# sonbui25/Multimodal-Aspect-Category-Sentiment-Analysis

Hardware: AMD Instinct MI355X
Metric: train samples/sec (fwd+bwd+step) FCMF seq128x36ROI (higher is better)
Workload: dtype bf16; 1 GPU; FCMF-base fine-tune step, BASELINE configs[1]: batch 64 reviews x 6 aspects per GPU, seq 128, 7 images x (49 patches + 36 ROIs), precomputed ResNet-152 features, dropout 0.1, clip 1.0 + 4-group AdamW + linear schedule; global_batch=64, per_gpu_batch=64, seq_len=128, parallelism=dp1, sample_unit=1 review = 6 aspect forwards

## Files before the change

### multimodal-aspect-category-sentiment-analysis_amd/csrc/norm.hip

```cpp
#include "common.h"

constexpr int LN_MAXP = 8;

template <typename T, int NP>
__global__ __launch_bounds__(256) void add_ln_fwd_kernel(const T* __restrict__ x, const T* __restrict__ res,
                                                         int64_t res_stride, const float* __restrict__ gamma,
                                                         const float* __restrict__ beta, T* __restrict__ y,
                                                         T* __restrict__ z, float* __restrict__ mean,
                                                         float* __restrict__ rstd, int rows, int H, float eps,
                                                         float p, uint64_t seed, unsigned char* __restrict__ q8 = nullptr,
                                                         float* __restrict__ qscale = nullptr) {
  const int lane = threadIdx.x & 63;
  const float inv_keep = p > 0.f ? 1.0f / (1.0f - p) : 1.0f;
  typedef typename Vec4<T>::raw Raw;
  const int stride = gridDim.x * 4;
  int row = blockIdx.x * 4 + (threadIdx.x >> 6);
  Raw nx[NP], nr[NP];
  auto fetch = [&](int r) {
    if (r < rows) {
#pragma unroll
      for (int i = 0; i < NP; ++i) {
        const int c = (i * 64 + lane) * 4;
        if (c < H) {
          nx[i] = Vec4<T>::load_raw(x + (int64_t)r * H + c);
          if (res) nr[i] = Vec4<T>::load_raw(res + (int64_t)r * res_stride + c);
        }
      }
    }
  };
  fetch(row);
  for (; row < rows; row += stride) {
  Raw cx[NP], cr[NP];
#pragma unroll
  for (int i = 0; i < NP; ++i) { cx[i] = nx[i]; cr[i] = nr[i]; }
  fetch(row + stride);
  float4 v[NP];
  float s = 0.f;
#pragma unroll
  for (int i = 0; i < NP; ++i) {
    const int c = (i * 64 + lane) * 4;
    if (c < H) {
      float4 a = Vec4<T>::cvt(cx[i]);
      if (p > 0.f) {
        const uint64_t base = (uint64_t)row * H + c;
        float dm[4];
        dropout_mult4(seed, base, p, inv_keep, dm);
        a.x *= dm[0]; a.y *= dm[1]; a.z *= dm[2]; a.w *= dm[3];
      }
      if (res) {
        float4 r = Vec4<T>::cvt(cr[i]);
        a.x += r.x; a.y += r.y; a.z += r.z; a.w += r.w;
      }
      v[i] = a;
      s += a.x + a.y + a.z + a.w;
    }
  }
  const float mu = wave_sum(s) / (float)H;
  float q = 0.f;
#pragma unroll
  for (int i = 0; i < NP; ++i) {
    const int c = (i * 64 + lane) * 4;
    if (c < H) {
      float dx = v[i].x - mu, dy = v[i].y - mu, dz = v[i].z - mu, dw = v[i].w - mu;
      q += dx * dx + dy * dy + dz * dz + dw * dw;
    }
  }
  const float rs = rsqrtf(wave_sum(q) / (float)H + eps);
  if (lane == 0) { mean[row] = mu; rstd[row] = rs; }
  float amax = 0.f;
#pragma unroll
  for (int i = 0; i < NP; ++i) {
    const int c = (i * 64 + lane) * 4;
    if (c < H) {
      if (z) Vec4<T>::store(z + (int64_t)row * H + c, v[i]);
      const float4 g = *reinterpret_cast<const float4*>(gamma + c);
      const float4 b = *reinterpret_cast<const float4*>(beta + c);
      float4 o;
      o.x = (v[i].x - mu) * rs * g.x + b.x; o.y = (v[i].y - mu) * rs * g.y + b.y;
      o.z = (v[i].z - mu) * rs * g.z + b.z; o.w = (v[i].w - mu) * rs * g.w + b.w;
      Vec4<T>::store(y + (int64_t)row * H + c, o);
      if (q8) {
        o.x = to_f32<T>(from_f32<T>(o.x)); o.y = to_f32<T>(from_f32<T>(o.y)); o.z = to_f32<T>(from_f32<T>(o.z)); o.w = to_f32<T>(from_f32<T>(o.w));
        v[i] = o;
        amax = fmaxf(amax, fmaxf(fmaxf(fabsf(o.x), fabsf(o.y)), fmaxf(fabsf(o.z), fabsf(o.w))));
      }
    }
  }
  if (q8) {
    amax = wave_max(amax);
    const float sc = amax > 0.f ? amax * (1.0f / 448.0f) : 1.0f, inv = 1.0f / sc;
    if (lane == 0) qscale[row] = sc;
#pragma unroll
    for (int i = 0; i < NP; ++i) {
      const int c = (i * 64 + lane) * 4;
      if (c < H) {
        int w8 = 0;
        w8 = __builtin_amdgcn_cvt_pk_fp8_f32(v[i].x * inv, v[i].y * inv, w8, false);
        w8 = __builtin_amdgcn_cvt_pk_fp8_f32(v[i].z * inv, v[i].w * inv, w8, true);
        *reinterpret_cast<int*>(q8 + (int64_t)row * H + c) = w8;
      }
    }
  }
  }
}

template <typename T, int NP>
__global__ __launch_bounds__(256) void add_ln_bwd_kernel(const T* __restrict__ dy, const T* __restrict__ z,
                                                         const float* __restrict__ gamma,
                                                         const float* __restrict__ mean,
                                                         const float* __restrict__ rstd, T* __restrict__ dz,
                                                         T* __restrict__ dx, float* __restrict__ dgamma,
                                                         float* __restrict__ dbeta, float* __restrict__ dxsum,
                                                         float* __restrict__ partial, int rows, int H, float p,
                                                         uint64_t seed, unsigned char* __restrict__ q8 = nullptr,
                                                         float* __restrict__ qscale = nullptr) {
  __shared__ float4 red[2][3][NP][64];
  const int lane = threadIdx.x & 63, w = threadIdx.x >> 6;
  const float inv_keep = p > 0.f ? 1.0f / (1.0f - p) : 1.0f;
  float4 ag[NP], ab[NP], gm[NP], ax[NP];
#pragma unroll
  for (int i = 0; i < NP; ++i) {
    ag[i] = make_float4(0, 0, 0, 0); ab[i] = make_float4(0, 0, 0, 0); ax[i] = make_float4(0, 0, 0, 0);
    const int c = (i * 64 + lane) * 4;
    gm[i] = c < H ? *reinterpret_cast<const float4*>(gamma + c) : make_float4(0, 0, 0, 0);
  }
  typedef typename Vec4<T>::raw Raw;
  const int stride = gridDim.x * 4;
  int row = blockIdx.x * 4 + w;
  Raw nd[NP], nz[NP];
  float nmu = 0.f, nrs = 0.f;
  auto fetch = [&](int r) {
    if (r < rows) {
      nmu = mean[r]; nrs = rstd[r];
#pragma unroll
      for (int i = 0; i < NP; ++i) {
        const int c = (i * 64 + lane) * 4;
        if (c < H) { nd[i] = Vec4<T>::load_raw(dy + (int64_t)r * H + c); nz[i] = Vec4<T>::load_raw(z + (int64_t)r * H + c); }
      }
    }
  };
  fetch(row);
  for (; row < rows; row += stride) {
    const float mu = nmu, rs = nrs;
    Raw cd[NP], cz[NP];
#pragma unroll
    for (int i = 0; i < NP; ++i) { cd[i] = nd[i]; cz[i] = nz[i]; }
    fetch(row + stride);
    float4 gy[NP], xh[NP];
    float s1 = 0.f, s2 = 0.f;
#pragma unroll
    for (int i = 0; i < NP; ++i) {
      const int c = (i * 64 + lane) * 4;
      if (c < H) {
        const float4 d = Vec4<T>::cvt(cd[i]);
        const float4 zz = Vec4<T>::cvt(cz[i]);
        float4 h; h.x = (zz.x - mu) * rs; h.y = (zz.y - mu) * rs; h.z = (zz.z - mu) * rs; h.w = (zz.w - mu) * rs;
        ag[i].x += d.x * h.x; ag[i].y += d.y * h.y; ag[i].z += d.z * h.z; ag[i].w += d.w * h.w;
        ab[i].x += d.x; ab[i].y += d.y; ab[i].z += d.z; ab[i].w += d.w;
        float4 g; g.x = d.x * gm[i].x; g.y = d.y * gm[i].y; g.z = d.z * gm[i].z; g.w = d.w * gm[i].w;
        gy[i] = g; xh[i] = h;
        s1 += g.x + g.y + g.z + g.w;
        s2 += g.x * h.x + g.y * h.y + g.z * h.z + g.w * h.w;
      }
    }
    s1 = wave_sum(s1) / (float)H;
    s2 = wave_sum(s2) / (float)H;
#pragma unroll
    for (int i = 0; i < NP; ++i) {
      const int c = (i * 64 + lane) * 4;
      if (c < H) {
        float4 o;
        o.x = rs * (gy[i].x - s1 - xh[i].x * s2); o.y = rs * (gy[i].y - s1 - xh[i].y * s2);
        o.z = rs * (gy[i].z - s1 - xh[i].z * s2); o.w = rs * (gy[i].w - s1 - xh[i].w * s2);
        Vec4<T>::store(dz + (int64_t)row * H + c, o);
        if (dx) {
          const uint64_t base = (uint64_t)row * H + c;
          float dm[4];
          dropout_mult4(seed, base, p, inv_keep, dm);
          o.x *= dm[0]; o.y *= dm[1]; o.z *= dm[2]; o.w *= dm[3];
          Vec4<T>::store(dx + (int64_t)row * H + c, o);
        }
        ax[i].x += o.x; ax[i].y += o.y; ax[i].z += o.z; ax[i].w += o.w;
        if (q8) {
          o.x = to_f32<T>(from_f32<T>(o.x)); o.y = to_f32<T>(from_f32<T>(o.y)); o.z = to_f32<T>(from_f32<T>(o.z)); o.w = to_f32<T>(from_f32<T>(o.w));
          gy[i] = o;
        }
      }
    }
    if (q8) {
      float amax = 0.f;
#pragma unroll
      for (int i = 0; i < NP; ++i)
        if ((i * 64 + lane) * 4 < H) amax = fmaxf(amax, fmaxf(fmaxf(fabsf(gy[i].x), fabsf(gy[i].y)), fmaxf(fabsf(gy[i].z), fabsf(gy[i].w))));
      amax = wave_max(amax);
      const float sc = amax > 0.f ? amax * (1.0f / 448.0f) : 1.0f, inv = 1.0f / sc;
      if (lane == 0) qscale[row] = sc;
#pragma unroll
      for (int i = 0; i < NP; ++i) {
        const int c = (i * 64 + lane) * 4;
        if (c < H) {
          int w8 = 0;
          w8 = __builtin_amdgcn_cvt_pk_fp8_f32(gy[i].x * inv, gy[i].y * inv, w8, false);
          w8 = __builtin_amdgcn_cvt_pk_fp8_f32(gy[i].z * inv, gy[i].w * inv, w8, true);
          *reinterpret_cast<int*>(q8 + (int64_t)row * H + c) = w8;
        }
      }
    }
  }
#pragma unroll
  for (int step = 0; step < 2; ++step) {
    const int half = step == 0 ? 2 : 1;
    if (w >= half && w < 2 * half) {
#pragma unroll
      for (int i = 0; i < NP; ++i) { red[w - half][0][i][lane] = ag[i]; red[w - half][1][i][lane] = ab[i]; red[w - half][2][i][lane] = ax[i]; }
    }
    __syncthreads();
    if (w < half) {
#pragma unroll
      for (int i = 0; i < NP; ++i) {
        float4 a = red[w][0][i][lane], b = red[w][1][i][lane], c2 = red[w][2][i][lane];
        ag[i].x += a.x; ag[i].y += a.y; ag[i].z += a.z; ag[i].w += a.w;
        ab[i].x += b.x; ab[i].y += b.y; ab[i].z += b.z; ab[i].w += b.w;
        ax[i].x += c2.x; ax[i].y += c2.y; ax[i].z += c2.z; ax[i].w += c2.w;
      }
    }
    __syncthreads();
  }
  if (w == 0) {
#pragma unroll
    for (int i = 0; i < NP; ++i) {
      const int c = (i * 64 + lane) * 4;
      if (c < H) {
        if (partial) {
          float* pb = partial + (int64_t)blockIdx.x * 3 * H + c;
          *reinterpret_cast<float4*>(pb) = ag[i];
          *reinterpret_cast<float4*>(pb + H) = ab[i];
          *reinterpret_cast<float4*>(pb + 2 * H) = ax[i];
        } else {
          atomicAdd(dgamma + c + 0, ag[i].x); atomicAdd(dgamma + c + 1, ag[i].y);
          atomicAdd(dgamma + c + 2, ag[i].z); atomicAdd(dgamma + c + 3, ag[i].w);
          atomicAdd(dbeta + c + 0, ab[i].x); atomicAdd(dbeta + c + 1, ab[i].y);
          atomicAdd(dbeta + c + 2, ab[i].z); atomicAdd(dbeta + c + 3, ab[i].w);
          if (dxsum) {
            atomicAdd(dxsum + c + 0, ax[i].x); atomicAdd(dxsum + c + 1, ax[i].y);
            atomicAdd(dxsum + c + 2, ax[i].z); atomicAdd(dxsum + c + 3, ax[i].w);
          }
        }
      }
    }
  }
}

__global__ __launch_bounds__(256) void ln_partial_reduce_kernel(const float* __restrict__ partial, int nblocks, int H,
                                                                float* __restrict__ dgamma, float* __restrict__ dbeta,
                                                                float* __restrict__ dxsum) {
  __shared__ float red[4][64];
  const int lane = threadIdx.x & 63, w = threadIdx.x >> 6;
  const int col = blockIdx.x * 64 + lane, which = blockIdx.y;
  float* out = which == 0 ? dgamma : (which == 1 ? dbeta : dxsum);
  if (!out) return;
  const int per = (nblocks + gridDim.z - 1) / gridDim.z;
  const int b0 = blockIdx.z * per, b1 = min(nblocks, b0 + per);
  float s = 0.f;
  if (col < H)
    for (int b = b0 + w; b < b1; b += 4) s += partial[((int64_t)b * 3 + which) * H + col];
  red[w][lane] = s;
  __syncthreads();
  if (w == 0 && col < H) atomicAdd(out + col, red[0][lane] + red[1][lane] + red[2][lane] + red[3][lane]);
}

__global__ __launch_bounds__(64) void position_ids_kernel(const int64_t* __restrict__ ids, int64_t* __restrict__ pos,
                                                          int S, int pad_id) {
  const int lane = threadIdx.x;
  const int64_t* row = ids + (int64_t)blockIdx.x * S;
  int64_t* out = pos + (int64_t)blockIdx.x * S;
  int running = 0;
  for (int t0 = 0; t0 < S; t0 += 64) {
    const int t = t0 + lane;
    const bool nz = t < S && row[t] != pad_id;
    const unsigned long long b = __ballot(nz);
    const int incl = __popcll(b & ((lane == 63) ? ~0ull : ((1ull << (lane + 1)) - 1)));
    if (t < S) out[t] = nz ? (int64_t)(running + incl + pad_id) : (int64_t)pad_id;
    running += __popcll(b);
  }
}

template <typename T, int NP>
__global__ __launch_bounds__(256) void embed_ln_fwd_kernel(const int64_t* __restrict__ ids, const int64_t* __restrict__ pos,
                                                           const int64_t* __restrict__ tt, const float* __restrict__ word,
                                                           const float* __restrict__ ptab, const float* __restrict__ ttab,
                                                           const float* __restrict__ gamma, const float* __restrict__ beta,
                                                           T* __restrict__ y, T* __restrict__ z, float* __restrict__ mean,
                                                           float* __restrict__ rstd, int ntok, int H, float eps, float p,
                                                           uint64_t seed) {
  const int lane = threadIdx.x & 63;
  const int row = blockIdx.x * 4 + (threadIdx.x >> 6);
  if (row >= ntok) return;
  const float* wr = word + ids[row] * H;
  const float* pr = ptab + pos[row] * H;
  const float* tr = ttab + (tt ? tt[row] : 0) * H;
  float4 v[NP];
  float s = 0.f;
#pragma unroll
  for (int i = 0; i < NP; ++i) {
    const int c = (i * 64 + lane) * 4;
    if (c < H) {
      const float4 a = *reinterpret_cast<const float4*>(wr + c);
      const float4 b = *reinterpret_cast<const float4*>(tr + c);
      const float4 d = *reinterpret_cast<const float4*>(pr + c);
      float4 o; o.x = (a.x + b.x) + d.x; o.y = (a.y + b.y) + d.y; o.z = (a.z + b.z) + d.z; o.w = (a.w + b.w) + d.w;
      v[i] = o;
      s += o.x + o.y + o.z + o.w;
    }
  }
  const float mu = wave_sum(s) / (float)H;
  float q = 0.f;
#pragma unroll
  for (int i = 0; i < NP; ++i) {
    const int c = (i * 64 + lane) * 4;
    if (c < H) {
      float dx = v[i].x - mu, dy = v[i].y - mu, dz = v[i].z - mu, dw = v[i].w - mu;
      q += dx * dx + dy * dy + dz * dz + dw * dw;
    }
  }
  const float rs = rsqrtf(wave_sum(q) / (float)H + eps);
  if (lane == 0) { mean[row] = mu; rstd[row] = rs; }
  const float inv_keep = p > 0.f ? 1.0f / (1.0f - p) : 1.0f;
#pragma unroll
  for (int i = 0; i < NP; ++i) {
    const int c = (i * 64 + lane) * 4;
    if (c < H) {
      if (z) Vec4<T>::store(z + (int64_t)row * H + c, v[i]);
      const float4 g = *reinterpret_cast<const float4*>(gamma + c);
      const float4 b = *reinterpret_cast<const float4*>(beta + c);
      float4 o;
      o.x = (v[i].x - mu) * rs * g.x + b.x; o.y = (v[i].y - mu) * rs * g.y + b.y;
      o.z = (v[i].z - mu) * rs * g.z + b.z; o.w = (v[i].w - mu) * rs * g.w + b.w;
      if (p > 0.f) {
        const uint64_t base = (uint64_t)row * H + c;
        float dm[4];
        dropout_mult4(seed, base, p, inv_keep, dm);
        o.x *= dm[0]; o.y *= dm[1]; o.z *= dm[2]; o.w *= dm[3];
      }
      Vec4<T>::store(y + (int64_t)row * H + c, o);
    }
  }
}

template <typename T>
__global__ __launch_bounds__(256) void embed_bwd_kernel(const T* __restrict__ dz, const int64_t* __restrict__ ids,
                                                        const int64_t* __restrict__ pos, const int64_t* __restrict__ tt,
                                                        float* __restrict__ dword, float* __restrict__ dpos,
                                                        float* __restrict__ dtt, int ntok, int H, int pad_id) {
  const int lane = threadIdx.x & 63;
  const int row = blockIdx.x * 4 + (threadIdx.x >> 6);
  if (row >= ntok) return;
  const int64_t id = ids[row], ps = pos[row], ty = tt ? tt[row] : 0;
  for (int c = lane; c < H; c += 64) {
    const float d = to_f32<T>(dz[(int64_t)row * H + c]);
    if (id != pad_id) atomicAdd(dword + id * H + c, d);
    if (dpos && ps != pad_id) atomicAdd(dpos + ps * H + c, d);
    if (dtt && ty != 0) atomicAdd(dtt + ty * H + c, d);
  }
}

template <typename T>
__global__ __launch_bounds__(256) void embed_type0_kernel(const T* __restrict__ dz, const int64_t* __restrict__ tt,
                                                          float* __restrict__ dtt, int ntok, int H, int rows_per_block) {
  __shared__ float red[4][64];
  const int lane = threadIdx.x & 63, w = threadIdx.x >> 6;
  const int col = blockIdx.x * 64 + lane;
  const int r0 = blockIdx.y * rows_per_block, r1 = min(ntok, r0 + rows_per_block);
  float s = 0.f;
  if (col < H)
    for (int r = r0 + w; r < r1; r += 4)
      if (!tt || tt[r] == 0) s += to_f32<T>(dz[(int64_t)r * H + col]);
  red[w][lane] = s;
  __syncthreads();
  if (w == 0 && col < H) atomicAdd(dtt + col, red[0][lane] + red[1][lane] + red[2][lane] + red[3][lane]);
}

template <typename T>
__global__ __launch_bounds__(256) void embed_pos_bwd_kernel(const T* __restrict__ dz, const int64_t* __restrict__ pos,
                                                            float* __restrict__ dpos, int nseq, int S, int H, int pad_id) {
  const int s = blockIdx.x, c = blockIdx.y * 256 + threadIdx.x;
  if (c >= H) return;
  int64_t p0 = -1;
  float acc = 0.f;
  const int g0 = blockIdx.z * 64, g1 = min(nseq, g0 + 64);
#pragma unroll 8
  for (int g = g0; g < g1; ++g) {
    const int64_t row = (int64_t)g * S + s, id = pos[row];
    if (id == pad_id) continue;
    const float d = to_f32<T>(dz[row * H + c]);
    if (p0 < 0) p0 = id;
    if (id == p0) acc += d;
    else atomicAdd(dpos + id * H + c, d);
  }
  if (p0 >= 0) atomicAdd(dpos + p0 * H + c, acc);
}

template <typename T>
__global__ __launch_bounds__(256) void embed_pos_type_bwd_kernel(const T* __restrict__ dz, const int64_t* __restrict__ pos,
                                                                 const int64_t* __restrict__ tt, float* __restrict__ dpos,
                                                                 float* __restrict__ dtt, int nseq, int S, int H, int pad_id) {
  constexpr int E = 16 / (int)sizeof(T);
  typedef T VecT __attribute__((ext_vector_type(E)));
  extern __shared__ __attribute__((aligned(16))) float red[];
  const int CE = H / E, slots = 256 / CE;
  const int tid = threadIdx.x, cg = tid % CE, slot = tid / CE, c0 = cg * E;
  const int s = blockIdx.x, g0 = blockIdx.y * 64, g1 = min(nseq, g0 + 64);
  float* rp = red;
  float* rt = red + slots * H;
  int* p0s = reinterpret_cast<int*>(red + 2 * slots * H);
  if (slot < slots) {
    float acc[E], tsum[E];
#pragma unroll
    for (int j = 0; j < E; ++j) acc[j] = tsum[j] = 0.f;
    int64_t p0 = -1;
#pragma unroll 4
    for (int g = g0 + slot; g < g1; g += slots) {
      const int64_t row = (int64_t)g * S + s, id = pos[row], ty = tt ? tt[row] : 0;
      const VecT v = *reinterpret_cast<const VecT*>(dz + row * H + c0);
      if (dtt) {
        if (ty == 0) {
#pragma unroll
          for (int j = 0; j < E; ++j) tsum[j] += (float)v[j];
        } else {
#pragma unroll
          for (int j = 0; j < E; ++j) atomicAdd(dtt + ty * H + c0 + j, (float)v[j]);
        }
      }
      if (id == pad_id) continue;
      if (p0 < 0) p0 = id;
      if (id == p0) {
#pragma unroll
        for (int j = 0; j < E; ++j) acc[j] += (float)v[j];
      } else {
#pragma unroll
        for (int j = 0; j < E; ++j) atomicAdd(dpos + id * H + c0 + j, (float)v[j]);
      }
    }
#pragma unroll
    for (int j = 0; j < E; ++j) { rp[slot * H + c0 + j] = acc[j]; rt[slot * H + c0 + j] = tsum[j]; }
    if (cg == 0) p0s[slot] = (int)p0;
  }
  __syncthreads();
  for (int c = tid; c < H; c += 256) {
    float ts = 0.f;
    for (int k = 0; k < slots; ++k) ts += rt[k * H + c];
    if (dtt) atomicAdd(dtt + c, ts);
    for (int k = 0; k < slots; ++k) {
      const int pk = p0s[k];
      if (pk < 0) continue;
      bool first = true;
      for (int m = 0; m < k; ++m) first = first && p0s[m] != pk;
      if (!first) continue;
      float ps = 0.f;
      for (int m = k; m < slots; ++m)
        if (p0s[m] == pk) ps += rp[m * H + c];
      atomicAdd(dpos + (int64_t)pk * H + c, ps);
    }
  }
}

#define LN_DISPATCH_T(T, H)                         \
  do {                                              \
    const int np__ = ((H) + 255) / 256;             \
    if (np__ <= 1) LAUNCH_(T, 1);                   \
    else if (np__ <= 2) LAUNCH_(T, 2);              \
    else if (np__ <= 3) LAUNCH_(T, 3);              \
    else if (np__ <= 4) LAUNCH_(T, 4);              \
    else LAUNCH_(T, 8);                             \
  } while (0)
#define LN_DISPATCH(dtype, H)                                     \
  do {                                                            \
    if ((dtype) == FCMF_F32) LN_DISPATCH_T(float, H);             \
    else LN_DISPATCH_T(bf16_t, H);                                \
  } while (0)

static int add_ln_fwd_impl(const void* x, const void* res, int64_t res_stride, const float* gamma, const float* beta, void* y,
                           void* z, float* mean, float* rstd, int rows, int H, float eps, float dropout_p, uint64_t seed,
                           int dtype, void* stream, void* q8, float* qscale);
extern "C" int fcmf_add_ln_fwd(const void* x, const void* res, int64_t res_stride, const float* gamma,
                               const float* beta, void* y, void* z, float* mean, float* rstd, int rows, int H,
                               float eps, float dropout_p, uint64_t seed, int dtype, void* stream) {
  return add_ln_fwd_impl(x, res, res_stride, gamma, beta, y, z, mean, rstd, rows, H, eps, dropout_p, seed, dtype, stream, nullptr, nullptr);
}
extern "C" int fcmf_add_ln_fwd_fp8(const void* x, const void* res, int64_t res_stride, const float* gamma,
                                   const float* beta, void* y, void* z, float* mean, float* rstd, int rows, int H,
                                   float eps, float dropout_p, uint64_t seed, int dtype, void* q8, float* qscale, void* stream) {
  if (!q8 || !qscale) return FCMF_ERR_ARG;
  return add_ln_fwd_impl(x, res, res_stride, gamma, beta, y, z, mean, rstd, rows, H, eps, dropout_p, seed, dtype, stream, q8, qscale);
}
static int add_ln_fwd_impl(const void* x, const void* res, int64_t res_stride, const float* gamma, const float* beta, void* y,
                           void* z, float* mean, float* rstd, int rows, int H, float eps, float dropout_p, uint64_t seed,
                           int dtype, void* stream, void* q8, float* qscale) {
  if (!x || !gamma || !beta || !y || !mean || !rstd || rows < 0 || H <= 0) return FCMF_ERR_ARG;
  if (H % 4 != 0 || H > LN_MAXP * 256 || (res && res_stride % 4 != 0)) return FCMF_ERR_UNSUPPORTED;
  if (rows == 0) return FCMF_OK;
  hipStream_t st = reinterpret_cast<hipStream_t>(stream);
  const int nblk = (rows + 3) / 4;
  dim3 grid(nblk > 2048 ? 2048 : nblk);
  if (dtype != FCMF_F32 && dtype != FCMF_BF16) return FCMF_ERR_UNSUPPORTED;
#define LAUNCH_(T, NP) hipLaunchKernelGGL((add_ln_fwd_kernel<T, NP>), grid, dim3(256), 0, st, (const T*)x, (const T*)res, \
    res_stride, gamma, beta, (T*)y, (T*)z, mean, rstd, rows, H, eps, dropout_p, seed, (unsigned char*)q8, qscale)
  LN_DISPATCH(dtype, H);
#undef LAUNCH_
  FCMF_CHECK_LAUNCH();
  return FCMF_OK;
}

static int ln_bwd_blocks(int rows) {
  int blocks = (rows + 3) / 4;
  return blocks > 1024 ? 1024 : blocks;
}

extern "C" int64_t fcmf_add_ln_bwd_workspace(int rows, int H) { return (int64_t)ln_bwd_blocks(rows) * 3 * H; }

static int add_ln_bwd_impl(const void* dy, const void* z, const float* gamma, const float* mean, const float* rstd, void* dz,
                           void* dx, float* dgamma, float* dbeta, float* dxsum, float* workspace, int rows, int H,
                           float dropout_p, uint64_t seed, int dtype, void* stream, void* q8, float* qscale);
extern "C" int fcmf_add_ln_bwd(const void* dy, const void* z, const float* gamma, const float* mean, const float* rstd,
                               void* dz, void* dx, float* dgamma, float* dbeta, float* dxsum, float* workspace,
                               int rows, int H, float dropout_p, uint64_t seed, int dtype, void* stream) {
  return add_ln_bwd_impl(dy, z, gamma, mean, rstd, dz, dx, dgamma, dbeta, dxsum, workspace, rows, H, dropout_p, seed, dtype, stream, nullptr, nullptr);
}
extern "C" int fcmf_add_ln_bwd_fp8(const void* dy, const void* z, const float* gamma, const float* mean, const float* rstd,
                                   void* dz, void* dx, float* dgamma, float* dbeta, float* dxsum, float* workspace,
                                   int rows, int H, float dropout_p, uint64_t seed, int dtype, void* q8, float* qscale, void* stream) {
  if (!q8 || !qscale) return FCMF_ERR_ARG;
  return add_ln_bwd_impl(dy, z, gamma, mean, rstd, dz, dx, dgamma, dbeta, dxsum, workspace, rows, H, dropout_p, seed, dtype, stream, q8, qscale);
}
static int add_ln_bwd_impl(const void* dy, const void* z, const float* gamma, const float* mean, const float* rstd, void* dz,
                           void* dx, float* dgamma, float* dbeta, float* dxsum, float* workspace, int rows, int H,
                           float dropout_p, uint64_t seed, int dtype, void* stream, void* q8, float* qscale) {
  if (!dy || !z || !gamma || !mean || !rstd || !dz || !dgamma || !dbeta || rows < 0 || H <= 0) return FCMF_ERR_ARG;
  if (H % 4 != 0 || H > LN_MAXP * 256) return FCMF_ERR_UNSUPPORTED;
  if (dropout_p > 0.f && !dx) return FCMF_ERR_ARG;
  if (rows == 0) return FCMF_OK;
  hipStream_t st = reinterpret_cast<hipStream_t>(stream);
  const int blocks = ln_bwd_blocks(rows);
  if (dtype != FCMF_F32 && dtype != FCMF_BF16) return FCMF_ERR_UNSUPPORTED;
#define LAUNCH_(T, NP) hipLaunchKernelGGL((add_ln_bwd_kernel<T, NP>), dim3(blocks), dim3(256), 0, st, (const T*)dy, (const T*)z, \
    gamma, mean, rstd, (T*)dz, (T*)(dropout_p > 0.f ? dx : nullptr), dgamma, dbeta, dxsum, workspace, rows, H, dropout_p, seed, \
    (unsigned char*)q8, qscale)
  LN_DISPATCH(dtype, H);
#undef LAUNCH_
  if (workspace)
    hipLaunchKernelGGL(ln_partial_reduce_kernel, dim3((H + 63) / 64, 3, 8), dim3(256), 0, st, workspace, blocks, H, dgamma, dbeta, dxsum);
  FCMF_CHECK_LAUNCH();
  return FCMF_OK;
}

extern "C" int fcmf_position_ids(const int64_t* ids, int64_t* pos, int nseq, int S, int pad_id, void* stream) {
  if (!ids || !pos || nseq < 0 || S <= 0) return FCMF_ERR_ARG;
  if (nseq == 0) return FCMF_OK;
  hipLaunchKernelGGL(position_ids_kernel, dim3(nseq), dim3(64), 0, reinterpret_cast<hipStream_t>(stream), ids, pos, S, pad_id);
  FCMF_CHECK_LAUNCH();
  return FCMF_OK;
}

extern "C" int fcmf_embed_ln_fwd(const int64_t* ids, const int64_t* pos, const int64_t* type_ids, const float* word,
                                 const float* pos_table, const float* type_table, const float* gamma, const float* beta,
                                 void* y, void* z, float* mean, float* rstd, int ntok, int H, float eps, float dropout_p,
                                 uint64_t seed, int dtype, void* stream) {
  if (!ids || !pos || !word || !pos_table || !type_table || !gamma || !beta || !y || !mean || !rstd) return FCMF_ERR_ARG;
  if (H % 4 != 0 || H > LN_MAXP * 256) return FCMF_ERR_UNSUPPORTED;
  if (ntok <= 0) return ntok == 0 ? FCMF_OK : FCMF_ERR_ARG;
  hipStream_t st = reinterpret_cast<hipStream_t>(stream);
  dim3 grid((ntok + 3) / 4);
  if (dtype != FCMF_F32 && dtype != FCMF_BF16) return FCMF_ERR_UNSUPPORTED;
#define LAUNCH_(T, NP) hipLaunchKernelGGL((embed_ln_fwd_kernel<T, NP>), grid, dim3(256), 0, st, ids, pos, type_ids, word, \
    pos_table, type_table, gamma, beta, (T*)y, (T*)z, mean, rstd, ntok, H, eps, dropout_p, seed)
  LN_DISPATCH(dtype, H);
#undef LAUNCH_
  FCMF_CHECK_LAUNCH();
  return FCMF_OK;
}

extern "C" int fcmf_embed_bwd(const void* dz, const int64_t* ids, const int64_t* pos, const int64_t* type_ids, float* dword,
                              float* dpos, float* dtype_table, int ntok, int H, int pad_id, int dtype, void* stream) {
  if (!dz || !ids || !pos || !dword) return FCMF_ERR_ARG;
  if (H % 4 != 0) return FCMF_ERR_UNSUPPORTED;
  if (ntok <= 0) return ntok == 0 ? FCMF_OK : FCMF_ERR_ARG;
  hipStream_t st = reinterpret_cast<hipStream_t>(stream);
  dim3 grid((ntok + 3) / 4);
  const int rpb = 512;
  dim3 g2((H + 63) / 64, (ntok + rpb - 1) / rpb);
  if (dtype == FCMF_F32) {
    hipLaunchKernelGGL((embed_bwd_kernel<float>), grid, dim3(256), 0, st, (const float*)dz, ids, pos, type_ids, dword, dpos, dtype_table, ntok, H, pad_id);
    if (dtype_table) hipLaunchKernelGGL((embed_type0_kernel<float>), g2, dim3(256), 0, st, (const float*)dz, type_ids, dtype_table, ntok, H, rpb);
  } else if (dtype == FCMF_BF16) {
    hipLaunchKernelGGL((embed_bwd_kernel<bf16_t>), grid, dim3(256), 0, st, (const bf16_t*)dz, ids, pos, type_ids, dword, dpos, dtype_table, ntok, H, pad_id);
    if (dtype_table) hipLaunchKernelGGL((embed_type0_kernel<bf16_t>), g2, dim3(256), 0, st, (const bf16_t*)dz, type_ids, dtype_table, ntok, H, rpb);
  } else return FCMF_ERR_UNSUPPORTED;
  FCMF_CHECK_LAUNCH();
  return FCMF_OK;
}

extern "C" int fcmf_embed_pos_type_bwd(const void* dz, const int64_t* pos, const int64_t* type_ids, float* dpos, float* dtype_table,
                                       int nseq, int S, int H, int pad_id, int dtype, void* stream) {
  if (!dz || !pos || !dpos || nseq < 0 || S <= 0 || H <= 0) return FCMF_ERR_ARG;
  if (nseq == 0) return FCMF_OK;
  if (dtype != FCMF_F32 && dtype != FCMF_BF16) return FCMF_ERR_UNSUPPORTED;
  const int E = dtype == FCMF_F32 ? 4 : 8;
  if (H % E != 0 || H / E > 256 || (reinterpret_cast<uintptr_t>(dz) & 15)) return FCMF_ERR_UNSUPPORTED;
  hipStream_t st = reinterpret_cast<hipStream_t>(stream);
  const int slots = 256 / (H / E);
  const size_t smem = sizeof(float) * 2 * (size_t)slots * H + sizeof(int) * slots;
  dim3 grid(S, (nseq + 63) / 64);
  if (dtype == FCMF_F32) hipLaunchKernelGGL((embed_pos_type_bwd_kernel<float>), grid, dim3(256), smem, st, (const float*)dz, pos, type_ids, dpos, dtype_table, nseq, S, H, pad_id);
  else hipLaunchKernelGGL((embed_pos_type_bwd_kernel<bf16_t>), grid, dim3(256), smem, st, (const bf16_t*)dz, pos, type_ids, dpos, dtype_table, nseq, S, H, pad_id);
  FCMF_CHECK_LAUNCH();
  return FCMF_OK;
}

extern "C" int fcmf_embed_pos_bwd(const void* dz, const int64_t* pos, float* dpos, int nseq, int S, int H, int pad_id,
                                  int dtype, void* stream) {
  if (!dz || !pos || !dpos || nseq < 0 || S <= 0 || H <= 0) return FCMF_ERR_ARG;
  if (nseq == 0) return FCMF_OK;
  hipStream_t st = reinterpret_cast<hipStream_t>(stream);
  dim3 grid(S, (H + 255) / 256, (nseq + 63) / 64);
  if (dtype == FCMF_F32) hipLaunchKernelGGL((embed_pos_bwd_kernel<float>), grid, dim3(256), 0, st, (const float*)dz, pos, dpos, nseq, S, H, pad_id);
  else if (dtype == FCMF_BF16) hipLaunchKernelGGL((embed_pos_bwd_kernel<bf16_t>), grid, dim3(256), 0, st, (const bf16_t*)dz, pos, dpos, nseq, S, H, pad_id);
  else return FCMF_ERR_UNSUPPORTED;
  FCMF_CHECK_LAUNCH();
  return FCMF_OK;
}
```

Measured before the change: 1773 samples/s.

## Add two-rows-per-wave bf16x8 LayerNorm forward/backward kernels with occupancy-capped grids

Adds new bf16 add+LayerNorm forward and backward kernels in which each 64-lane wave handles two rows, one per 32-lane half, using 16-byte bf16x8 loads and stores and half-wave reductions. The backward kernel prefetches one or two rows ahead, accumulates dgamma/dbeta/dxsum partials in registers and combines them through shared memory. Grid size is capped at the number of resident blocks queried from the occupancy API, so the partial reduce runs with fewer blocks and a single z-slice. The aim is fewer, wider memory transactions and better latency hiding for H of 1024 or less. In exchange it adds alignment checks, more register pressure, and an FCMF_LN_V1 environment fallback to the old kernels.

```diff
diff --git a/multimodal-aspect-category-sentiment-analysis_amd/csrc/norm.hip b/multimodal-aspect-category-sentiment-analysis_amd/csrc/norm.hip
--- a/multimodal-aspect-category-sentiment-analysis_amd/csrc/norm.hip
+++ b/multimodal-aspect-category-sentiment-analysis_amd/csrc/norm.hip
@@ -269,6 +269,284 @@
   if (w == 0 && col < H) atomicAdd(out + col, red[0][lane] + red[1][lane] + red[2][lane] + red[3][lane]);
 }
 
+constexpr int LN2_MAXP = 4;
+#define LN2_BWD_DEPTH(NP, Q) (((NP) <= 3 && !(Q)) ? 2 : 1)
+
+__device__ __forceinline__ float half_sum(float v) {
+#pragma unroll
+  for (int o = 16; o > 0; o >>= 1) v += __shfl_xor(v, o, 64);
+  return v;
+}
+__device__ __forceinline__ float half_max(float v) {
+#pragma unroll
+  for (int o = 16; o > 0; o >>= 1) v = fmaxf(v, __shfl_xor(v, o, 64));
+  return v;
+}
+__device__ __forceinline__ void dropout_mult8(uint64_t seed, uint64_t base, float p, float inv_keep, float (&m)[8]) {
+  const uint32_t thr = dropout_threshold(p);
+  const uint64_t k0 = base >> 1;
+  const uint32_t lo = (uint32_t)k0, hi = (uint32_t)(k0 >> 32);
+  const uint32_t fold = (uint32_t)seed ^ ((hi << 7) | (hi >> 25)), s1 = (uint32_t)(seed >> 32);
+#pragma unroll
+  for (int j = 0; j < 4; ++j) {
+    const uint32_t h = fcmf_hash32_rounds((lo + j) ^ fold, s1);
+    m[2 * j] = (h & 0xFFFFu) >= thr ? inv_keep : 0.f;
+    m[2 * j + 1] = (h >> 16) >= thr ? inv_keep : 0.f;
+  }
+}
+__device__ __forceinline__ void store_bf16x8(bf16_t* p, const float (&v)[8]) {
+  bf16x8 o;
+#pragma unroll
+  for (int j = 0; j < 8; ++j) o[j] = (bf16_t)v[j];
+  *reinterpret_cast<bf16x8*>(p) = o;
+}
+__device__ __forceinline__ void store_fp8x8(unsigned char* p, const float (&v)[8], float inv) {
+  int w0 = 0, w1 = 0;
+  w0 = __builtin_amdgcn_cvt_pk_fp8_f32(v[0] * inv, v[1] * inv, w0, false);
+  w0 = __builtin_amdgcn_cvt_pk_fp8_f32(v[2] * inv, v[3] * inv, w0, true);
+  w1 = __builtin_amdgcn_cvt_pk_fp8_f32(v[4] * inv, v[5] * inv, w1, false);
+  w1 = __builtin_amdgcn_cvt_pk_fp8_f32(v[6] * inv, v[7] * inv, w1, true);
+  *reinterpret_cast<int2*>(p) = make_int2(w0, w1);
+}
+
+template <int NP, bool Q>
+__global__ __launch_bounds__(256) void add_ln_fwd_rows2_kernel(const bf16_t* x, const bf16_t* __restrict__ res,
+                                                               int64_t res_stride, const float* __restrict__ gamma,
+                                                               const float* __restrict__ beta, bf16_t* __restrict__ y,
+                                                               bf16_t* z, float* __restrict__ mean,
+                                                               float* __restrict__ rstd, int rows, int H, float eps,
+                                                               float p, uint64_t seed, unsigned char* __restrict__ q8,
+                                                               float* __restrict__ qscale) {
+  const int lane = threadIdx.x & 63, l = lane & 31, hf = lane >> 5;
+  const float inv_keep = p > 0.f ? 1.0f / (1.0f - p) : 1.0f;
+  const int npairs = (rows + 1) >> 1, stride = gridDim.x * 4;
+  int pr = blockIdx.x * 4 + (threadIdx.x >> 6);
+  bf16x8 x1[NP] = {}, r1[NP] = {}, x2[NP] = {}, r2[NP] = {};
+  auto fetch = [&](int64_t pp, bf16x8 (&fx)[NP], bf16x8 (&fr)[NP]) {
+    const int64_t r = 2 * pp + hf;
+    if (r < rows) {
+#pragma unroll
+      for (int i = 0; i < NP; ++i) {
+        const int c = (i * 32 + l) * 8;
+        if (c < H) {
+          fx[i] = *reinterpret_cast<const bf16x8*>(x + r * H + c);
+          if (res) fr[i] = *reinterpret_cast<const bf16x8*>(res + r * res_stride + c);
+        }
+      }
+    }
+  };
+  fetch(pr, x1, r1);
+  fetch((int64_t)pr + stride, x2, r2);
+  for (; pr < npairs; pr += stride) {
+    bf16x8 cx[NP], cr[NP];
+#pragma unroll
+    for (int i = 0; i < NP; ++i) { cx[i] = x1[i]; cr[i] = r1[i]; x1[i] = x2[i]; r1[i] = r2[i]; }
+    fetch((int64_t)pr + 2 * (int64_t)stride, x2, r2);
+    const int64_t row = 2 * (int64_t)pr + hf;
+    const bool valid = row < rows;
+    float v[NP][8];
+    float s = 0.f;
+#pragma unroll
+    for (int i = 0; i < NP; ++i) {
+      const int c = (i * 32 + l) * 8;
+      if (c < H) {
+        float a[8];
+#pragma unroll
+        for (int j = 0; j < 8; ++j) a[j] = (float)cx[i][j];
+        if (p > 0.f) {
+          float dm[8];
+          dropout_mult8(seed, (uint64_t)row * H + c, p, inv_keep, dm);
+#pragma unroll
+          for (int j = 0; j < 8; ++j) a[j] *= dm[j];
+        }
+        if (res) {
+#pragma unroll
+          for (int j = 0; j < 8; ++j) a[j] += (float)cr[i][j];
+        }
+        float t = a[0];
+#pragma unroll
+        for (int j = 0; j < 8; ++j) { v[i][j] = a[j]; if (j) t += a[j]; }
+        s += t;
+      }
+    }
+    const float mu = half_sum(s) / (float)H;
+    float q = 0.f;
+#pragma unroll
+    for (int i = 0; i < NP; ++i) {
+      if ((i * 32 + l) * 8 < H) {
+        float t = 0.f;
+#pragma unroll
+        for (int j = 0; j < 8; ++j) { const float d = v[i][j] - mu; t = j ? t + d * d : d * d; }
+        q += t;
+      }
+    }
+    const float rs = rsqrtf(half_sum(q) / (float)H + eps);
+    if (valid && l == 0) { mean[row] = mu; rstd[row] = rs; }
+    float amax = 0.f;
+#pragma unroll
+    for (int i = 0; i < NP; ++i) {
+      const int c = (i * 32 + l) * 8;
+      if (c < H) {
+        if (z && valid) store_bf16x8(z + row * H + c, v[i]);
+        const float4 g0 = *reinterpret_cast<const float4*>(gamma + c), g1 = *reinterpret_cast<const float4*>(gamma + c + 4);
+        const float4 b0 = *reinterpret_cast<const float4*>(beta + c), b1 = *reinterpret_cast<const float4*>(beta + c + 4);
+        const float g[8] = {g0.x, g0.y, g0.z, g0.w, g1.x, g1.y, g1.z, g1.w};
+        const float b[8] = {b0.x, b0.y, b0.z, b0.w, b1.x, b1.y, b1.z, b1.w};
+        float o[8];
+#pragma unroll
+        for (int j = 0; j < 8; ++j) o[j] = (v[i][j] - mu) * rs * g[j] + b[j];
+        if (valid) store_bf16x8(y + row * H + c, o);
+        if (Q) {
+#pragma unroll
+          for (int j = 0; j < 8; ++j) { v[i][j] = (float)(bf16_t)o[j]; amax = fmaxf(amax, fabsf(v[i][j])); }
+        }
+      }
+    }
+    if (Q) {
+      amax = half_max(amax);
+      const float sc = amax > 0.f ? amax * (1.0f / 448.0f) : 1.0f, inv = 1.0f / sc;
+      if (valid && l == 0) qscale[row] = sc;
+#pragma unroll
+      for (int i = 0; i < NP; ++i) {
+        const int c = (i * 32 + l) * 8;
+        if (c < H && valid) store_fp8x8(q8 + row * H + c, v[i], inv);
+      }
+    }
+  }
+}
+
+template <int NP, bool Q, int D>
+__global__ __launch_bounds__(256, NP <= 3 ? 2 : 1) void add_ln_bwd_rows2_kernel(const bf16_t* __restrict__ dy, const bf16_t* __restrict__ z,
+                                                               const float* __restrict__ gamma, const float* __restrict__ mean,
+                                                               const float* __restrict__ rstd, bf16_t* __restrict__ dz,
+                                                               bf16_t* __restrict__ dx, float* __restrict__ partial, int rows,
+                                                               int H, float p, uint64_t seed, unsigned char* __restrict__ q8,
+                                                               float* __restrict__ qscale) {
+  __shared__ float red[4][3][NP * 256];
+  const int lane = threadIdx.x & 63, l = lane & 31, hf = lane >> 5, w = threadIdx.x >> 6;
+  const float inv_keep = p > 0.f ? 1.0f / (1.0f - p) : 1.0f;
+  float ag[NP][8], ab[NP][8], ax[NP][8], gm[NP][8];
+#pragma unroll
+  for (int i = 0; i < NP; ++i) {
+    const int c = (i * 32 + l) * 8;
+    float4 g0 = make_float4(0, 0, 0, 0), g1 = g0;
+    if (c < H) { g0 = *reinterpret_cast<const float4*>(gamma + c); g1 = *reinterpret_cast<const float4*>(gamma + c + 4); }
+    gm[i][0] = g0.x; gm[i][1] = g0.y; gm[i][2] = g0.z; gm[i][3] = g0.w; gm[i][4] = g1.x; gm[i][5] = g1.y; gm[i][6] = g1.z; gm[i][7] = g1.w;
+#pragma unroll
+    for (int j = 0; j < 8; ++j) ag[i][j] = ab[i][j] = ax[i][j] = 0.f;
+  }
+  const int npairs = (rows + 1) >> 1, stride = gridDim.x * 4;
+  int pr = blockIdx.x * 4 + w;
+  bf16x8 d1[NP] = {}, z1[NP] = {}, d2[NP] = {}, z2[NP] = {};
+  float mu1 = 0.f, rs1 = 0.f, mu2 = 0.f, rs2 = 0.f;
+  auto fetch = [&](int64_t pp, bf16x8 (&fd)[NP], bf16x8 (&fz)[NP], float& fmu, float& frs) {
+    const int64_t r = 2 * pp + hf;
+    if (r < rows) {
+      fmu = mean[r]; frs = rstd[r];
+#pragma unroll
+      for (int i = 0; i < NP; ++i) {
+        const int c = (i * 32 + l) * 8;
+        if (c < H) {
+          fd[i] = *reinterpret_cast<const bf16x8*>(dy + r * H + c);
+          fz[i] = *reinterpret_cast<const bf16x8*>(z + r * H + c);
+        }
+      }
+    }
+  };
+  fetch(pr, d1, z1, mu1, rs1);
+  if (D == 2) fetch((int64_t)pr + stride, d2, z2, mu2, rs2);
+  for (; pr < npairs; pr += stride) {
+    const float mu = mu1, rs = rs1;
+    bf16x8 cd[NP], cz[NP];
+#pragma unroll
+    for (int i = 0; i < NP; ++i) { cd[i] = d1[i]; cz[i] = z1[i]; }
+    if (D == 2) {
+#pragma unroll
+      for (int i = 0; i < NP; ++i) { d1[i] = d2[i]; z1[i] = z2[i]; }
+      mu1 = mu2; rs1 = rs2;
+      fetch((int64_t)pr + 2 * (int64_t)stride, d2, z2, mu2, rs2);
+    } else {
+      fetch((int64_t)pr + stride, d1, z1, mu1, rs1);
+    }
+    const int64_t row = 2 * (int64_t)pr + hf;
+    const bool valid = row < rows;
+    float s1 = 0.f, s2 = 0.f;
+#pragma unroll
+    for (int i = 0; i < NP; ++i) {
+      if ((i * 32 + l) * 8 < H && valid) {
+        float t1 = 0.f, t2 = 0.f;
+#pragma unroll
+        for (int j = 0; j < 8; ++j) {
+          const float d = (float)cd[i][j];
+          const float h = ((float)cz[i][j] - mu) * rs;
+          ag[i][j] += d * h;
+          ab[i][j] += d;
+          const float g = d * gm[i][j];
+          t1 = j ? t1 + g : g;
+          t2 = j ? t2 + g * h : g * h;
+        }
+        s1 += t1; s2 += t2;
+      }
+    }
+    s1 = half_sum(s1) / (float)H;
+    s2 = half_sum(s2) / (float)H;
+    float amax = 0.f;
+    float qv[Q ? NP : 1][8];
+#pragma unroll
+    for (int i = 0; i < NP; ++i) {
+      const int c = (i * 32 + l) * 8;
+      if (c < H && valid) {
+        float o[8];
+#pragma unroll
+        for (int j = 0; j < 8; ++j) {
+          const float h = ((float)cz[i][j] - mu) * rs;
+          o[j] = rs * ((float)cd[i][j] * gm[i][j] - s1 - h * s2);
+        }
+        store_bf16x8(dz + row * H + c, o);
+        if (dx) {
+          float dm[8];
+          dropout_mult8(seed, (uint64_t)row * H + c, p, inv_keep, dm);
+#pragma unroll
+          for (int j = 0; j < 8; ++j) o[j] *= dm[j];
+          store_bf16x8(dx + row * H + c, o);
+        }
+#pragma unroll
+        for (int j = 0; j < 8; ++j) ax[i][j] += o[j];
+        if (Q) {
+#pragma unroll
+          for (int j = 0; j < 8; ++j) { qv[i][j] = (float)(bf16_t)o[j]; amax = fmaxf(amax, fabsf(qv[i][j])); }
+        }
+      }
+    }
+    if (Q) {
+      amax = half_max(amax);
+      const float sc = amax > 0.f ? amax * (1.0f / 448.0f) : 1.0f, inv = 1.0f / sc;
+      if (valid && l == 0) qscale[row] = sc;
+#pragma unroll
+      for (int i = 0; i < NP; ++i) {
+        const int c = (i * 32 + l) * 8;
+        if (c < H && valid) store_fp8x8(q8 + row * H + c, qv[Q ? i : 0], inv);
+      }
+    }
+  }
+#pragma unroll
+  for (int i = 0; i < NP; ++i) {
+#pragma unroll
+    for (int j = 0; j < 8; ++j) {
+      const float a = ag[i][j] + __shfl_xor(ag[i][j], 32, 64), b = ab[i][j] + __shfl_xor(ab[i][j], 32, 64),
+                  c2 = ax[i][j] + __shfl_xor(ax[i][j], 32, 64);
+      if (hf == 0) {
+        const int c = (i * 32 + l) * 8 + j;
+        red[w][0][c] = a; red[w][1][c] = b; red[w][2][c] = c2;
+      }
+    }
+  }
+  __syncthreads();
+  float* pb = partial + (int64_t)blockIdx.x * 3 * H;
+  for (int k = 0; k < 3; ++k)
+    for (int c = threadIdx.x; c < H; c += 256) pb[k * H + c] = ((red[0][k][c] + red[1][k][c]) + red[2][k][c]) + red[3][k][c];
+}
+
 __global__ __launch_bounds__(64) void position_ids_kernel(const int64_t* __restrict__ ids, int64_t* __restrict__ pos,
                                                           int S, int pad_id) {
   const int lane = threadIdx.x;
@@ -479,6 +757,26 @@
     else LN_DISPATCH_T(bf16_t, H);                                \
   } while (0)
 
+static bool ln_rows2_shape(int H) {
+  static const bool v1 = [] { const char* e = getenv("FCMF_LN_V1"); return e && e[0] == '1'; }();
+  return !v1 && H % 8 == 0 && H <= LN2_MAXP * 256;
+}
+template <class K> static int ln_resident_blocks(K kernel, int fallback) {
+  int dev = 0, cus = 0, per = 0;
+  if (hipGetDevice(&dev) != hipSuccess || hipDeviceGetAttribute(&cus, hipDeviceAttributeMultiprocessorCount, dev) != hipSuccess ||
+      hipOccupancyMaxActiveBlocksPerMultiprocessor(&per, kernel, 256, 0) != hipSuccess || cus <= 0 || per <= 0)
+    return fallback;
+  return cus * per;
+}
+static bool ln_al16(const void* p) { return (reinterpret_cast<uintptr_t>(p) & 15) == 0; }
+#define LN2_DISPATCH(H, Q)                          \
+  do {                                              \
+    const int np__ = ((H) + 255) / 256;             \
+    if (np__ <= 1) LAUNCH2_(1, Q);                  \
+    else if (np__ <= 2) LAUNCH2_(2, Q);             \
+    else if (np__ <= 3) LAUNCH2_(3, Q);             \
+    else LAUNCH2_(4, Q);                            \
+  } while (0)
 static int add_ln_fwd_impl(const void* x, const void* res, int64_t res_stride, const float* gamma, const float* beta, void* y,
                            void* z, float* mean, float* rstd, int rows, int H, float eps, float dropout_p, uint64_t seed,
                            int dtype, void* stream, void* q8, float* qscale);
@@ -503,6 +801,20 @@
   const int nblk = (rows + 3) / 4;
   dim3 grid(nblk > 2048 ? 2048 : nblk);
   if (dtype != FCMF_F32 && dtype != FCMF_BF16) return FCMF_ERR_UNSUPPORTED;
+  if (dtype == FCMF_BF16 && ln_rows2_shape(H) && ln_al16(x) && ln_al16(y) && ln_al16(z) && (!res || (ln_al16(res) && res_stride % 8 == 0)) &&
+      !(reinterpret_cast<uintptr_t>(q8) & 7)) {
+    const int nb = (rows + 7) / 8;
+#define LAUNCH2_(NP, Q) do {                                                                                                       \
+    static const int cap__ = ln_resident_blocks(add_ln_fwd_rows2_kernel<NP, Q>, 768);                                              \
+    hipLaunchKernelGGL((add_ln_fwd_rows2_kernel<NP, Q>), dim3(nb > cap__ ? cap__ : nb), dim3(256), 0, st, (const bf16_t*)x,        \
+    (const bf16_t*)res, res_stride, gamma, beta, (bf16_t*)y, (bf16_t*)z, mean, rstd, rows, H, eps, dropout_p, seed, (unsigned char*)q8, qscale); \
+  } while (0)
+    if (q8) LN2_DISPATCH(H, true);
+    else LN2_DISPATCH(H, false);
+#undef LAUNCH2_
+    FCMF_CHECK_LAUNCH();
+    return FCMF_OK;
+  }
 #define LAUNCH_(T, NP) hipLaunchKernelGGL((add_ln_fwd_kernel<T, NP>), grid, dim3(256), 0, st, (const T*)x, (const T*)res, \
     res_stride, gamma, beta, (T*)y, (T*)z, mean, rstd, rows, H, eps, dropout_p, seed, (unsigned char*)q8, qscale)
   LN_DISPATCH(dtype, H);
@@ -542,6 +854,24 @@
   hipStream_t st = reinterpret_cast<hipStream_t>(stream);
   const int blocks = ln_bwd_blocks(rows);
   if (dtype != FCMF_F32 && dtype != FCMF_BF16) return FCMF_ERR_UNSUPPORTED;
+  if (dtype == FCMF_BF16 && workspace && ln_rows2_shape(H) && ln_al16(dy) && ln_al16(z) && ln_al16(dz) && ln_al16(dx) &&
+      !(reinterpret_cast<uintptr_t>(q8) & 7)) {
+    const int nb = (rows + 7) / 8;
+    int b2 = nb > 1024 ? 1024 : nb;
+#define LAUNCH2_(NP, Q) do {                                                                                                       \
+    static const int cap__ = ln_resident_blocks(add_ln_bwd_rows2_kernel<NP, Q, LN2_BWD_DEPTH(NP, Q)>, 512);                        \
+    if (b2 > cap__) b2 = cap__;                                                                                                    \
+    hipLaunchKernelGGL((add_ln_bwd_rows2_kernel<NP, Q, LN2_BWD_DEPTH(NP, Q)>), dim3(b2), dim3(256), 0, st, (const bf16_t*)dy,      \
+    (const bf16_t*)z, gamma, mean, rstd, (bf16_t*)dz, (bf16_t*)(dropout_p > 0.f ? dx : nullptr), workspace, rows, H, dropout_p,   \
+    seed, (unsigned char*)q8, qscale);                                                                                             \
+  } while (0)
+    if (q8) LN2_DISPATCH(H, true);
+    else LN2_DISPATCH(H, false);
+#undef LAUNCH2_
+    hipLaunchKernelGGL(ln_partial_reduce_kernel, dim3((H + 63) / 64, 3, 1), dim3(256), 0, st, workspace, b2, H, dgamma, dbeta, dxsum);
+    FCMF_CHECK_LAUNCH();
+    return FCMF_OK;
+  }
 #define LAUNCH_(T, NP) hipLaunchKernelGGL((add_ln_bwd_kernel<T, NP>), dim3(blocks), dim3(256), 0, st, (const T*)dy, (const T*)z, \
     gamma, mean, rstd, (T*)dz, (T*)(dropout_p > 0.f ? dx : nullptr), dgamma, dbeta, dxsum, workspace, rows, H, dropout_p, seed, \
     (unsigned char*)q8, qscale)
```

Result: slower. 1755 samples/s (-1.1%).
